# CSU-KangHu/HiTE

Hardware: AMD Instinct MI355X
Metric: candidate TE boundaries/sec on 1 Gbp synthetic genome (fine stage: copy finding+gather+align+vote+judge) (higher is better)
Workload: dtype u8; 1 GPU; C3: 1000 Mbp synthetic genome, 2500 TIR + 2500 LTR families, 50000 candidates/GPU judged as TIR (copy finding by minimizer-index lookup inside the timed step; index build 0.0 s untimed); genome_bp=1000000000, candidates_per_gpu=50000, candidate_bases=192511237, copies=799813, copy_table=found, is_te=34225, parallelism=replicated genome, candidates per rank x1, all-gather of 32-B calls

## Files before the change

hite_amd/csrc/hite_align.hip:

```cpp
#include "hite_common.h"
#include "hite_scan.h"
#include "hite_arena.h"
#include "hite_sort.h"
#include "hite_align.h"

#define AL_GAP 3
#define AL_STEER 24
#define AL_MARGIN 48
#define AL_PADR 1056
#define AL_WIDE_NW 64
#define AL_STRIP 16
#define AL_RECB 4096
#define AL_DEFAULT_CAP 8
#define AL_KBINS 2048
#define AL_LANES_MIN_STRIPS 32

struct AlignArgs {
    const uint8_t *win;
    const int64_t *win_off;
    const int32_t *win_len;
    const int32_t *row_first;
    int n_cand;
    const int32_t *row_cand;
    const uint4 *planes;
// ... 353 lines not shown
                    const int tr = m - H;
                    if (t + s > tr) s = (tr - t) & ~3;
                    const int need = tr - 3 - 8 * ((n - j) >> 2) - t;
                    if (s < need) s = (need + 3) & ~3;
                    if (s > 8) { status = 2; act = false; s = 8; }
                    if (!half) {
                        stop += plane_sum(X2[0], X1[0], X0[0], (1u << s) - 1u) - AL_GAP * s;
                        brec[(cc >> 2) * 2] = (uint32_t)(s >> 2) | (i2 << 2) | (i1 << 10) | (i0 << 18);
                    }
#pragma unroll
                    for (int w = 0; w < HW - 1; w++) {
                        X2[w] = alignbit(X2[w + 1], X2[w], (uint32_t)s); X1[w] = alignbit(X1[w + 1], X1[w], (uint32_t)s);
                        X0[w] = alignbit(X0[w + 1], X0[w], (uint32_t)s);
                        A0[w] = alignbit(A0[w + 1], A0[w], (uint32_t)s); A1[w] = alignbit(A1[w + 1], A1[w], (uint32_t)s);
                        AN[w] = alignbit(AN[w + 1], AN[w], (uint32_t)s);
                    }
                    X2[HW - 1] = alignbit(half ? 0xffffffffu : u2, X2[HW - 1], (uint32_t)s);
                    X1[HW - 1] = alignbit(half ? 0xffffffffu : u1, X1[HW - 1], (uint32_t)s);
                    X0[HW - 1] = alignbit(half ? 0u : u0, X0[HW - 1], (uint32_t)s);
                    A0[HW - 1] = alignbit(half ? f0 : ua0, A0[HW - 1], (uint32_t)s);
                    A1[HW - 1] = alignbit(half ? f1 : ua1, A1[HW - 1], (uint32_t)s);
                    AN[HW - 1] = alignbit(half ? fn : uan, AN[HW - 1], (uint32_t)s);
                    f0 >>= s; f1 >>= s; fn >>= s;
                    t += s;
                    if (t >= 1) { const int v = t + 1 - j; LO = v > LO ? v : LO; }
                    if (t + W < m) { const int jl = j + 3 < n ? j + 3 : n; const int v = t + W - jl; HI = v < HI ? v : HI; }
                }
            }
            const uint32_t word = cc < 4 ? bw.x : (cc < 8 ? bw.y : (cc < 12 ? bw.z : bw.w));
            const BaseMask bm = base_mask((word >> (8 * (cc & 3))) & 0xffu);
            uint32_t Bv[HW], Pv[HW], Yv[HW], Sv[HW], eqv[HW], vposv[HW];
#pragma unroll
            for (int w = 0; w < HW; w++) {
                eqv[w] = ~((A0[w] ^ bm.m0) | (A1[w] ^ bm.m1) | AN[w] | bm.inv);
                vposv[w] = X2[w] & X1[w];
                Bv[w] = eqv[w] | ~(X2[w] | X1[w] | X0[w]);
            }
            const uint32_t pvpos = pair_partner(vposv[HW - 1]);
            const uint32_t vin = half ? pvpos >> 31 : 0u;
            uint32_t cin = 0u, tap0 = 0u;
#pragma unroll
            for (int w = 0; w < HW; w++) {
                if (w == HW - 1) tap0 = cin;
                Pv[w] = (vposv[w] << 1) | (w ? vposv[w - 1] >> 31 : vin);
                Yv[w] = Pv[w] | Bv[w];
                unsigned cout;
                Sv[w] = __builtin_addc(Bv[w], Yv[w], cin, &cout);
                cin = cout;
            }
            {
                const uint32_t pc = pair_partner(cin);
                uint32_t e = half ? pc : 0u;
#pragma unroll
                for (int w = 0; w < HW; w++) { const uint32_t o = Sv[w]; Sv[w] = o + e; e &= (o == 0xffffffffu) ? 1u : 0u; }
            }
            uint32_t Zv[HW], h2v[HW], h1v[HW], h0v[HW];
#pragma unroll
            for (int w = 0; w < HW; w++) {
                Zv[w] = Bv[w] | (Pv[w] & (Sv[w] ^ Bv[w] ^ Yv[w]));
                const uint32_t b1 = Zv[w] & X0[w], b2 = X1[w] & b1;
                h0v[w] = ~(Zv[w] ^ X0[w]); h1v[w] = ~(X1[w] ^ b1); h2v[w] = ~(X2[w] ^ b2);
            }
            const uint32_t q2 = pair_partner(h2v[HW - 1]) >> 31, q1 = pair_partner(h1v[HW - 1]) >> 31, q0 = pair_partner(h0v[HW - 1]) >> 31;
            const uint32_t hin2 = half ? q2 : 1u, hin1 = half ? q1 : 1u, hin0 = half ? q0 : 0u;
            if (on) {
#pragma unroll
                for (int w = 0; w < HW; w++) {
                    const uint32_t s2 = (h2v[w] << 1) | (w ? h2v[w - 1] >> 31 : hin2), s1 = (h1v[w] << 1) | (w ? h1v[w - 1] >> 31 : hin1),
                                   s0 = (h0v[w] << 1) | (w ? h0v[w - 1] >> 31 : hin0);
                    const uint32_t c1 = Zv[w] & s0, c2 = s1 & c1;
                    X0[w] = ~(Zv[w] ^ s0); X1[w] = ~(s1 ^ c1); X2[w] = ~(s2 ^ c2);
                }
                if (!half) {
                    stop += AL_GAP;
                    const uint32_t c5 = tap0 | ((vposv[HW - 2] >> 31) << 1) | ((h2v[HW - 2] >> 31) << 2) | ((h1v[HW - 2] >> 31) << 3) | ((h0v[HW - 2] >> 31) << 4);
                    const int sh = 26 + 5 * (cc & 3);
                    if (sh + 5 <= 32) brec[(cc >> 2) * 2] |= c5 << sh;
                    else if (sh >= 32) brec[(cc >> 2) * 2 + 1] |= c5 << (sh - 32);
                    else { brec[(cc >> 2) * 2] |= c5 << sh; brec[(cc >> 2) * 2 + 1] |= c5 >> (32 - sh); }
                    brec[(cc >> 2) * 2 + 1] |= ((bm.m0 & 1u) | (bm.m1 & 2u) | (bm.inv & 4u)) << (14 + 3 * (cc & 3));
                }
            }
        }
        if (sa && !half) {
            uint4 *bp = reinterpret_cast<uint4 *>(rec0 + (size_t)k * AL_RECB + AL_RECB / 2);
            bp[0] = make_uint4(brec[0], brec[1], brec[2], brec[3]);
            bp[1] = make_uint4(brec[4], brec[5], brec[6], brec[7]);
        }
    }
    {
        const int extra = m - H - t;
        const uint32_t part = pair_partner((uint32_t)plane_sum(X2[0], X1[0], X0[0], (1u << (extra & 31)) - 1u));
        if (n > 0 && !half) {
            int U = -1, kstar = -1;
            if (status == 0) {
                int u = stop - AL_GAP * H;
#pragma unroll
                for (int w = 0; w < HW; w++) u += plane_sum(X2[w], X1[w], X0[w], 0xffffffffu);
                u += (int)part - AL_GAP * extra;
                U = u;
                const int d = m - n, dmin = d < 0 ? d : 0, dmax = d > 0 ? d : 0, ad = d < 0 ? -d : d;
                int E = dmin - LO;
                if (HI - dmax < E) E = HI - dmax;
                if (E > (1 << 27)) kstar = 0x7fffffff;
                else if (E >= 0) kstar = AL_GAP * ad + 2 * AL_GAP * E + 2 * AL_GAP - 1;
            }
            P.U[g] = U; P.kst[g] = kstar; P.st[g] = status; P.lvl[g] = NW;
        }
    }
}

template <int CTRL>
__device__ __forceinline__ uint32_t dpp_row(uint32_t v) { return (uint32_t)__builtin_amdgcn_update_dpp(0, (int)v, CTRL, 0xf, 0xf, true); }
template <int G>
__device__ __forceinline__ int grp_sum(int v) {
    v += (int)dpp_row<0xB1>((uint32_t)v);
    v += (int)dpp_row<0x4E>((uint32_t)v);
    if (G == 8) v += (int)dpp_row<0x141>((uint32_t)v);
    return v;
}
__device__ __forceinline__ int wave_min_i32(int v) {
#pragma unroll
    for (int d = 32; d >= 1; d >>= 1) { int o = __shfl_xor(v, d, 64); v = o < v ? o : v; }
    return v;
}
__device__ __forceinline__ uint32_t bit_mask(uint32_t w, int bit) { return (uint32_t)((int32_t)(w << (31 - bit)) >> 31); }
template <int GI>
__device__ __forceinline__ uint32_t quad_bcast(uint32_t v) { return dpp_row<GI * 0x55>(v); }
struct LaneFwd {
    uint32_t X2, X1, X0, A0, A1, AN, f0, f1, fn;
    int t, stop, LO, HI, status;
    bool act;
};
template <int G, bool FULL>
__device__ __forceinline__ void lanes_strip(LaneFwd &S, const uint4 bw, const uint32_t invm, const uint32_t code12, const bool sa, const int k,
                                            const int m, const int n, const int q, const uint32_t K1, const unsigned long long TOPM, uint32_t (&brec)[8]) {
    constexpr int NW = G, W = 32 * NW, H = W / 2, S0 = NW / 2 - 1;
    const bool top = q == G - 1;
#pragma unroll
    for (int cc = 0; cc < AL_STRIP; cc++) {
        const int j = k * AL_STRIP + cc + 1;
        const bool on = FULL || (sa && j <= n);
        if ((cc & 3) == 0) {
            const int ds = grp_sum<G>((q == S0 || q == S0 + 1) ? slope_count(S.X2, S.X1, S.X0) : 0);
            const uint32_t i2 = dpp_row<0x102>(S.X2) & 0xffu, i1 = dpp_row<0x102>(S.X1) & 0xffu, i0 = dpp_row<0x102>(S.X0) & 0xffu;
            const uint32_t u2 = dpp_row<0x101>(S.X2), u1 = dpp_row<0x101>(S.X1), u0 = dpp_row<0x101>(S.X0);
            const uint32_t ua0 = dpp_row<0x101>(S.A0), ua1 = dpp_row<0x101>(S.A1), uan = dpp_row<0x101>(S.AN);
            constexpr int gi = 0;
            const uint32_t cg = (cc >> 2) == 0 ? quad_bcast<0>(code12) : ((cc >> 2) == 1 ? quad_bcast<1>(code12) : ((cc >> 2) == 2 ? quad_bcast<2>(code12) : quad_bcast<3>(code12)));
            (void)gi;
            if (on) {
                int s = ds > AL_STEER ? 0 : (ds < -AL_STEER ? 8 : 4);
                const int tr = m - H;
                if (S.t + s > tr) s = (tr - S.t) & ~3;
                const int need = tr - 3 - 8 * ((n - j) >> 2) - S.t;
                if (s < need) s = (need + 3) & ~3;
                if (s > 8) { S.status = 2; S.act = false; s = 8; }
                S.stop += plane_sum(S.X2, S.X1, S.X0, (1u << s) - 1u) - AL_GAP * s;
                brec[(cc >> 2) * 2] = (uint32_t)(s >> 2) | (i2 << 2) | (i1 << 10) | (i0 << 18);
                brec[(cc >> 2) * 2 + 1] = cg << 14;
                S.X2 = alignbit(top ? 0xffffffffu : u2, S.X2, (uint32_t)s);
                S.X1 = alignbit(top ? 0xffffffffu : u1, S.X1, (uint32_t)s);
                S.X0 = alignbit(top ? 0u : u0, S.X0, (uint32_t)s);
                S.A0 = alignbit(top ? S.f0 : ua0, S.A0, (uint32_t)s);
                S.A1 = alignbit(top ? S.f1 : ua1, S.A1, (uint32_t)s);
                S.AN = alignbit(top ? S.fn : uan, S.AN, (uint32_t)s);
                S.f0 >>= s; S.f1 >>= s; S.fn >>= s;
                S.t += s;
                if (S.t >= 1) { const int v = S.t + 1 - j; S.LO = v > S.LO ? v : S.LO; }
                if (S.t + W < m) { const int jl = j + 3 < n ? j + 3 : n; const int v = S.t + W - jl; S.HI = v < S.HI ? v : S.HI; }
            }
        }
        const uint32_t word = cc < 4 ? bw.x : (cc < 8 ? bw.y : (cc < 12 ? bw.z : bw.w));
        const uint32_t m0 = bit_mask(word, 8 * (cc & 3) + 1), m1 = bit_mask(word, 8 * (cc & 3) + 2), inv = bit_mask(invm, cc);
        const uint32_t eq = ~((S.A0 ^ m0) | (S.A1 ^ m1) | S.AN | inv);
        const uint32_t vpos = S.X2 & S.X1;
        const uint32_t B = eq | ~(S.X2 | S.X1 | S.X0);
        const uint32_t pvr = dpp_row<0x111>(vpos);
        const uint32_t Pp = alignbit(vpos, pvr, 31) & ~K1;
        const uint32_t Y = Pp | B;
        unsigned long long Gm;
        const uint32_t sum0 = add_co_mask(B, Y, Gm);
        uint32_t sum;
        {
            const unsigned long long Pm = __ballot(sum0 == 0xffffffffu);
            const unsigned long long Gc = Gm & ~TOPM, Yy = (Pm | Gm) & ~TOPM, ss = Gc + Yy;
            sum = add_mask_bit(sum0, ss ^ Gc ^ Yy);
        }
        const uint32_t Z = B | (Pp & (sum ^ B ^ Y));
        const uint32_t h0 = ~(Z ^ S.X0), b1 = Z & S.X0, h1 = ~(S.X1 ^ b1), b2 = S.X1 & b1, h2 = ~(S.X2 ^ b2);
        const uint32_t r2 = dpp_row<0x111>(h2), r1 = dpp_row<0x111>(h1), r0 = dpp_row<0x111>(h0);
        if (on) {
            const uint32_t s2 = alignbit(h2, r2, 31) | K1, s1 = alignbit(h1, r1, 31) | K1, s0 = alignbit(h0, r0, 31) & ~K1;
            const uint32_t c1 = Z & s0, c2 = s1 & c1;
            S.X0 = ~(Z ^ s0); S.X1 = ~(s1 ^ c1); S.X2 = ~(s2 ^ c2);
            uint32_t c5 = alignbit(r0 >> 31, r1, 31);
            c5 = alignbit(c5, r2, 31);
            c5 = alignbit(c5, pvr, 31);
            c5 = (c5 << 1) | (sum - sum0);
            const int sh = 26 + 5 * (cc & 3);
            if (sh + 5 <= 32) brec[(cc >> 2) * 2] |= c5 << sh;
            else if (sh >= 32) brec[(cc >> 2) * 2 + 1] |= c5 << (sh - 32);
            else { brec[(cc >> 2) * 2] |= c5 << sh; brec[(cc >> 2) * 2 + 1] |= c5 >> (32 - sh); }
        }
    }
}
__device__ __forceinline__ uint32_t decode_bases4(uint32_t w) {
    uint32_t r = 0;
#pragma unroll
    for (int x = 0; x < 4; x++) {
        const unsigned ch = (w >> (8 * x)) & 0xffu;
        const uint32_t bad = is_acgt_byte(ch) ? 0u : 1u;
        r |= (bad << x) | ((((ch >> 1) & 3u) | (bad << 2)) << (4 + 3 * x));
    }
    return r;
}
template <int G>
__global__ void __launch_bounds__(64) align_fwd_lanes_kernel(AlignArgs P, const int32_t *__restrict__ list, int nlist) {
    constexpr int NW = G, W = 32 * NW, H = W / 2, S0 = NW / 2 - 1, PPW = 64 / G;
    const int q = threadIdx.x & (G - 1);
    const int li = blockIdx.x * PPW + (int)(threadIdx.x / G);
    const int g = li < nlist ? list[li] : -1;
    int m = 0, n = 0, g0 = 0, c = 0;
    if (g >= 0) {
        c = P.row_cand[g];
        g0 = P.row_first[c];
        if (g != g0) { m = P.win_len[g0]; n = P.win_len[g]; }
    }
    const int nmax = wave_max_i32(n);
    if (nmax == 0) return;
    const int nfull = wave_min_i32(n > 0 ? n : 0x7fffffff);
    const bool wr = q == S0;
    const uint32_t K1 = q == 0 ? 1u : 0u;
    const unsigned long long TOPM = G == 4 ? 0x8888888888888888ull : 0x8080808080808080ull;
    const uint8_t *b = P.win + (g >= 0 ? P.win_off[g] : 0);
    const uint4 *pl = P.planes + (g >= 0 ? P.plane_off[c] : 0);
    char *rec0 = g >= 0 ? reinterpret_cast<char *>(P.rec[g]) : nullptr;
    LaneFwd S;
    S.X2 = q >= NW / 2 ? 0xffffffffu : 0u; S.X1 = S.X2; S.X0 = 0u; S.A0 = 0u; S.A1 = 0u; S.AN = 0xffffffffu;
    S.f0 = S.f1 = S.fn = 0u;
    S.t = -H;
    S.act = n > 0;
    if (S.act) { const uint4 v = pl[((S.t + AL_PADR) >> 5) + q]; S.A0 = v.x; S.A1 = v.y; S.AN = v.z; }
    S.stop = AL_GAP * H; S.LO = -(1 << 28); S.HI = 1 << 28; S.status = 0;
    int fq = (S.t + W + AL_PADR) >> 5;
    uint4 Wa = make_uint4(0, 0, 0xffffffffu, 0), Wb = Wa, Wc = Wa, bnext = make_uint4(0, 0, 0, 0);
    if (S.act) { Wa = pl[fq]; Wb = pl[fq + 1]; Wc = pl[fq + 2]; bnext = *reinterpret_cast<const uint4 *>(b); }
    for (int k = 0; k * AL_STRIP < nmax; k++) {
        const bool sa = S.act && k * AL_STRIP < n;
        uint4 bw = make_uint4(0, 0, 0, 0);
        uint32_t brec[8] = {0, 0, 0, 0, 0, 0, 0, 0};
        {
            const uint32_t p2 = dpp_row<0x101>(S.X2), p1 = dpp_row<0x101>(S.X1), p0 = dpp_row<0x101>(S.X0);
            if (sa && wr) {
                uint4 *ck = reinterpret_cast<uint4 *>(rec0 + (size_t)k * AL_RECB);
                ck[0] = make_uint4(S.X2, p2, S.X1, p1);
                ck[1] = make_uint4(S.X0, p0, (uint32_t)(S.t + 32 * S0), 0u);
            }
        }
        S.f0 = S.f1 = S.fn = 0u;
        if (sa) {
            bw = bnext;
            if ((k + 1) * AL_STRIP < n) bnext = *reinterpret_cast<const uint4 *>(b + (k + 1) * AL_STRIP);
            const int fx = S.t + W + AL_PADR;
            if ((fx >> 5) != fq) { Wa = Wb; Wb = Wc; fq++; Wc = pl[fq + 2]; }
            const uint32_t sh = (uint32_t)fx & 31u;
            S.f0 = alignbit(Wb.x, Wa.x, sh); S.f1 = alignbit(Wb.y, Wa.y, sh); S.fn = alignbit(Wb.z, Wa.z, sh);
        }
        const uint32_t dq = (q & 3) == 0 ? bw.x : ((q & 3) == 1 ? bw.y : ((q & 3) == 2 ? bw.z : bw.w));
        const uint32_t dec = decode_bases4(dq);
        uint32_t invm = (dec & 15u) << (4 * (q & 3));
        invm |= dpp_row<0xB1>(invm);
        invm |= dpp_row<0x4E>(invm);
        const bool failed = __any(n > 0 && S.status != 0);
        if ((k + 1) * AL_STRIP <= nfull && !failed) lanes_strip<G, true>(S, bw, invm, dec >> 4, sa, k, m, n, q, K1, TOPM, brec);
        else lanes_strip<G, false>(S, bw, invm, dec >> 4, sa, k, m, n, q, K1, TOPM, brec);
        if (sa && wr) {
            uint4 *bp = reinterpret_cast<uint4 *>(rec0 + (size_t)k * AL_RECB + AL_RECB / 2);
            bp[0] = make_uint4(brec[0], brec[1], brec[2], brec[3]);
            bp[1] = make_uint4(brec[4], brec[5], brec[6], brec[7]);
        }
    }
    {
        const int extra = m - H - S.t;
        const int part = q < NW / 2 ? plane_sum(S.X2, S.X1, S.X0, 0xffffffffu) : (q == NW / 2 ? plane_sum(S.X2, S.X1, S.X0, (1u << (extra & 31)) - 1u) : 0);
        const int tot = grp_sum<G>(part + (q == 0 ? S.stop : 0));
        if (n > 0 && wr) {
            int U = -1, kstar = -1;
            if (S.status == 0) {
                U = tot + AL_GAP * n - AL_GAP * H - AL_GAP * extra;
                const int d = m - n, dmin = d < 0 ? d : 0, dmax = d > 0 ? d : 0, ad = d < 0 ? -d : d;
                int E = dmin - S.LO;
                if (S.HI - dmax < E) E = S.HI - dmax;
                if (E > (1 << 27)) kstar = 0x7fffffff;
                else if (E >= 0) kstar = AL_GAP * ad + 2 * AL_GAP * E + 2 * AL_GAP - 1;
            }
            P.U[g] = U; P.kst[g] = kstar; P.st[g] = S.status; P.lvl[g] = NW;
            if (NW == 4) P.U4[g] = U;
        }
    }
}

typedef unsigned int tb_u32x4 __attribute__((ext_vector_type(4)));
#if defined(ALIGN_TB_STORE8)
struct OpsOut {
    uint16_t *ops;
    unsigned long long acc, top;
    int m;
    __device__ __forceinline__ void init(uint16_t *row, int m_) { ops = row; m = m_; acc = 0ull; top = 0ull; }
    __device__ __forceinline__ void push(int pos, uint32_t val) {
        acc = (acc << 16) | (unsigned long long)(val & 0xffffu);
        if ((pos & 3) == 0) {
            if (pos + 4 <= m) *reinterpret_cast<unsigned long long *>(ops + pos) = acc;
            else top = acc;
        }
    }
    __device__ __forceinline__ void finish() {
        const int k = m & 3, p0 = m & ~3;
        for (int x = 0; x < k; x++) ops[p0 + x] = (uint16_t)(top >> (16 * x));
    }
};
#elif defined(ALIGN_TB_STORE32)
struct OpsOut {
    uint16_t *ops;
    unsigned long long acc;
    unsigned long long g0, g1, g2, g3;
    int m, off;
    int q_low;
    __device__ __forceinline__ void init(uint16_t *row, int m_) {
        ops = row; m = m_; acc = 0ull; g0 = g1 = g2 = g3 = 0ull;
        off = (int)((reinterpret_cast<uintptr_t>(row) >> 1) & 15);
        q_low = m_ + off;
    }
    __device__ __forceinline__ uint16_t held(int q, int q_acc_low) const {
        if ((q >> 2) == (q_acc_low >> 2) && (q_acc_low & 3)) return (uint16_t)(acc >> (16 * (q - q_acc_low)));
        const int g = (q >> 2) & 3;
        const unsigned long long s = g == 0 ? g0 : (g == 1 ? g1 : (g == 2 ? g2 : g3));
        return (uint16_t)(s >> (16 * (q & 3)));
    }
    __device__ __forceinline__ void push(int pos, uint32_t val) {
        acc = (acc << 16) | (unsigned long long)(val & 0xffffu);
        const int q = pos + off;
        if ((q & 3) == 0) {
            const int g = (q >> 2) & 3;
            g0 = g == 0 ? acc : g0; g1 = g == 1 ? acc : g1; g2 = g == 2 ? acc : g2; g3 = g == 3 ? acc : g3;
            if (g == 0) {
                if (pos + 16 <= m) {
                    tb_u32x4 *dst = reinterpret_cast<tb_u32x4 *>(ops + pos);
                    tb_u32x4 v0, v1;
                    v0.x = (unsigned)g0; v0.y = (unsigned)(g0 >> 32); v0.z = (unsigned)g1; v0.w = (unsigned)(g1 >> 32);
                    v1.x = (unsigned)g2; v1.y = (unsigned)(g2 >> 32); v1.z = (unsigned)g3; v1.w = (unsigned)(g3 >> 32);
                    dst[0] = v0; dst[1] = v1;
                } else {
                    for (int x = pos; x < m; x++) ops[x] = held(x + off, q);
                }
                q_low = q;
            }
        }
    }
    __device__ __forceinline__ void finish() {
        const int top = q_low - off < m ? q_low - off : m;
        for (int x = 0; x < top; x++) ops[x] = held(x + off, off);
    }
};

#else
struct OpsOut {
    uint16_t *ops;
    unsigned long long acc, hi;
    unsigned long long tacc, thi;
    int m, off;
    __device__ __forceinline__ void init(uint16_t *row, int m_) {
        ops = row; m = m_; acc = 0ull; hi = 0ull; tacc = 0ull; thi = 0ull;
        off = (int)((reinterpret_cast<uintptr_t>(row) >> 1) & 7);
    }
    __device__ __forceinline__ void push(int pos, uint32_t val) {
        acc = (acc << 16) | (unsigned long long)(val & 0xffffu);
        const int q = pos + off;
        if ((q & 3) == 0) {
            if (q & 4) hi = acc;
            else if (pos + 8 <= m) {
                tb_u32x4 v;
                v.x = (unsigned)acc; v.y = (unsigned)(acc >> 32); v.z = (unsigned)hi; v.w = (unsigned)(hi >> 32);
                *reinterpret_cast<tb_u32x4 *>(ops + pos) = v;
            } else { tacc = acc; thi = hi; }
        }
    }
    __device__ __forceinline__ void finish() {
        const int t0 = m - ((m + off) & 7);
        if (t0 >= 0) for (int x = t0; x < m; x++) { const int qq = x + off; ops[x] = (uint16_t)(((qq & 4) ? thi : tacc) >> (16 * (qq & 3))); }
        const int b0 = (8 - off) & 7;
        const int lowm = b0 < m ? b0 : m;
        for (int x = 0; x < lowm; x++) {
            const int qq = x + off;
            const bool in_acc = (off & 3) != 0 && (qq >> 2) == (off >> 2);
            ops[x] = in_acc ? (uint16_t)(acc >> (16 * x)) : (uint16_t)(hi >> (16 * (qq & 3)));
        }
    }
};
#endif

#ifdef ALIGN_TB_OCC
#define ALIGN_TB_ATTR __attribute__((amdgpu_waves_per_eu(ALIGN_TB_OCC, ALIGN_TB_OCC)))
#else
#define ALIGN_TB_ATTR
#endif
__global__ void __launch_bounds__(64) ALIGN_TB_ATTR align_tb_kernel(AlignArgs P, const int32_t *__restrict__ list, int nlist) {
    ACLK_BEGIN(1);
    const int li = blockIdx.x * 64 + threadIdx.x;
    const int g = li < nlist ? list[li] : -1;
    int m = 0, n = 0, g0 = 0, c = 0;
    if (g >= 0) {
        c = P.row_cand[g];
        g0 = P.row_first[c];
        if (g != g0 && P.st[g] == 0) { m = P.win_len[g0]; n = P.win_len[g]; }
    }
    const int nmax = wave_max_i32(n);
    if (nmax == 0) return;
    const uint4 *pl = P.planes + (g >= 0 ? P.plane_off[c] : 0);
    const char *rec0 = g >= 0 ? reinterpret_cast<const char *>(P.rec[g]) : nullptr;
    uint16_t *ops = P.ops + (g >= 0 ? P.ops_base[c] + (int64_t)(g - g0) * (m + 1) : 0);
    int i = m, j = n;
    bool fail = false;
    OpsOut out;
    out.init(ops, m);
    const int Kmax = (nmax + AL_STRIP - 1) / AL_STRIP;
    const int K = (n + AL_STRIP - 1) / AL_STRIP;
    struct Pw { uint32_t x, y, z; };
    uint4 ckA0, ckA1, ckB0, ckB1, bdA0, bdA1;
    Pw plA[4];
    ckA0 = ckA1 = ckB0 = ckB1 = bdA0 = bdA1 = make_uint4(0, 0, 0, 0);
#pragma unroll
    for (int w = 0; w < 4; w++) { plA[w].x = 0; plA[w].y = 0; plA[w].z = 0; }
    {
        const int k = Kmax - 1;
        if (k < K) {
            const uint4 *ck = reinterpret_cast<const uint4 *>(rec0 + (size_t)k * AL_RECB);
            ckA0 = ck[0]; ckA1 = ck[1];
            const uint4 *bp = reinterpret_cast<const uint4 *>(rec0 + (size_t)k * AL_RECB + AL_RECB / 2);
            bdA0 = bp[0]; bdA1 = bp[1];
            const int q0 = ((int)ckA1.z + AL_PADR) >> 5;
#pragma unroll
            for (int w = 0; w < 4; w++) { const uint4 v = pl[q0 + w]; plA[w].x = v.x; plA[w].y = v.y; plA[w].z = v.z; }
        }
        if (k >= 1 && k - 1 < K) {
            const uint4 *ck = reinterpret_cast<const uint4 *>(rec0 + (size_t)(k - 1) * AL_RECB);
            ckB0 = ck[0]; ckB1 = ck[1];
        }
    }
    for (int k = Kmax - 1; k >= 0; k--) {
        const bool sa = n > 0 && !fail && i > 0 && k < K;
        uint4 ckC0 = make_uint4(0, 0, 0, 0), ckC1 = ckC0, bdB0 = ckC0, bdB1 = ckC0;
        Pw plB[4];
#pragma unroll
        for (int w = 0; w < 4; w++) { plB[w].x = 0; plB[w].y = 0; plB[w].z = 0; }
        if (k >= 1 && k - 1 < K && !fail && i > 0) {
            const uint4 *bp = reinterpret_cast<const uint4 *>(rec0 + (size_t)(k - 1) * AL_RECB + AL_RECB / 2);
            bdB0 = bp[0]; bdB1 = bp[1];
            const int q0 = ((int)ckB1.z + AL_PADR) >> 5;
#pragma unroll
            for (int w = 0; w < 4; w++) { const uint4 v = pl[q0 + w]; plB[w].x = v.x; plB[w].y = v.y; plB[w].z = v.z; }
        }
        if (k >= 2 && k - 2 < K && !fail && i > 0) {
            const uint4 *ck = reinterpret_cast<const uint4 *>(rec0 + (size_t)(k - 2) * AL_RECB);
            ckC0 = ck[0]; ckC1 = ck[1];
        }
        if (__any(sa)) {
        uint32_t X2[2], X1[2], X0[2], A0[2], A1[2], AN[2];
        uint32_t f0 = 0, f1 = 0, fn = 0;
        uint32_t brec[8] = {0, 0, 0, 0, 0, 0, 0, 0};
        int t = 0;
        if (sa) {
            X2[0] = ckA0.x; X2[1] = ckA0.y; X1[0] = ckA0.z; X1[1] = ckA0.w; X0[0] = ckA1.x; X0[1] = ckA1.y;
            t = (int)ckA1.z;
            brec[0] = bdA0.x; brec[1] = bdA0.y; brec[2] = bdA0.z; brec[3] = bdA0.w;
            brec[4] = bdA1.x; brec[5] = bdA1.y; brec[6] = bdA1.z; brec[7] = bdA1.w;
            const uint32_t sh = (uint32_t)(t + AL_PADR) & 31u;
#pragma unroll
            for (int w = 0; w < 2; w++) {
                A0[w] = alignbit(plA[w + 1].x, plA[w].x, sh); A1[w] = alignbit(plA[w + 1].y, plA[w].y, sh);
                AN[w] = alignbit(plA[w + 1].z, plA[w].z, sh);
            }
            f0 = alignbit(plA[3].x, plA[2].x, sh); f1 = alignbit(plA[3].y, plA[2].y, sh); fn = alignbit(plA[3].z, plA[2].z, sh);
        } else {
#pragma unroll
            for (int w = 0; w < 2; w++) { X2[w] = 0; X1[w] = 0; X0[w] = 0; A0[w] = 0; A1[w] = 0; AN[w] = 0; }
        }
        unsigned long long dg[AL_STRIP], up[AL_STRIP];
        uint32_t sbits = 0;
#pragma unroll
        for (int cc = 0; cc < AL_STRIP; cc++) {
            const int jc = k * AL_STRIP + cc + 1;
            dg[cc] = 0ull; up[cc] = 0ull;
            if (sa && jc <= n) {
                const uint32_t rlo = brec[(cc >> 2) * 2], rhi = brec[(cc >> 2) * 2 + 1];
                if ((cc & 3) == 0) {
                    const uint32_t s = (rlo & 3u) << 2;
                    const uint32_t in2 = (rlo >> 2) & 0xffu, in1 = (rlo >> 10) & 0xffu, in0 = (rlo >> 18) & 0xffu;
                    X2[0] = alignbit(X2[1], X2[0], s); X1[0] = alignbit(X1[1], X1[0], s); X0[0] = alignbit(X0[1], X0[0], s);
                    A0[0] = alignbit(A0[1], A0[0], s); A1[0] = alignbit(A1[1], A1[0], s); AN[0] = alignbit(AN[1], AN[0], s);
                    X2[1] = alignbit(in2, X2[1], s); X1[1] = alignbit(in1, X1[1], s); X0[1] = alignbit(in0, X0[1], s);
                    A0[1] = alignbit(f0, A0[1], s); A1[1] = alignbit(f1, A1[1], s); AN[1] = alignbit(fn, AN[1], s);
                    f0 >>= s; f1 >>= s; fn >>= s;
                    t += (int)s;
                    sbits |= (rlo & 3u) << (2 * (cc >> 2));
                }
                const int sh = 26 + 5 * (cc & 3);
                const uint32_t c5 = (sh + 5 <= 32 ? rlo >> sh : (sh >= 32 ? rhi >> (sh - 32) : (rlo >> sh) | (rhi << (32 - sh)))) & 31u;
                const uint32_t code = rhi >> (14 + 3 * (cc & 3));
                BaseMask bm;
                bm.m0 = 0u - (code & 1u); bm.m1 = 0u - ((code >> 1) & 1u); bm.inv = 0u - ((code >> 2) & 1u);
                uint32_t tap[5], dgc[2], upc[2];
                bp_core<2, true, -1>(X2, X1, X0, A0, A1, AN, bm, c5 & 1u, (c5 >> 1) & 1u, (c5 >> 2) & 1u, (c5 >> 3) & 1u, (c5 >> 4) & 1u, dgc, upc, tap);
                dg[cc] = ((unsigned long long)dgc[1] << 32) | dgc[0];
                up[cc] = ((unsigned long long)upc[1] << 32) | upc[0];
            }
        }
        int tcur = t;
#pragma unroll
        for (int cc = AL_STRIP - 1; cc >= 0; cc--) {
            const int jc = k * AL_STRIP + cc + 1;
            if (sa && !fail && i > 0 && j == jc) {
                const int kb = i - tcur - 1;
                if ((unsigned)kb >= 64u) fail = true;
                else {
                    const unsigned long long stopm = (dg[cc] | ~up[cc]) & (0xffffffffffffffffull >> (63 - kb));
                    if (stopm == 0ull) fail = true;
                    else {
                        const int ps = 63 - __clzll(stopm);
                        int ups = kb - ps;
                        if (ups > i) ups = i;
                        const uint32_t gapv = (uint32_t)j | 0x8000u;
                        for (int x = 0; x < ups; x++) out.push(i - 1 - x, gapv);
                        i -= ups;
                        if (i > 0) {
                            if ((dg[cc] >> ps) & 1ull) { out.push(i - 1, (uint32_t)(j - 1)); i--; j--; }
                            else j--;
                        }
                    }
                }
            }
            if ((cc & 3) == 0) tcur -= (int)(((sbits >> (2 * (cc >> 2))) & 3u) << 2);
        }
        }
        ckA0 = ckB0; ckA1 = ckB1; ckB0 = ckC0; ckB1 = ckC1; bdA0 = bdB0; bdA1 = bdB1;
#pragma unroll
        for (int w = 0; w < 4; w++) plA[w] = plB[w];
    }
    if (n > 0) {
        if (fail) P.st[g] = 1;
        else {
            for (int q = i - 1; q >= 0; q--) out.push(q, 0x8000u);
            out.finish();
        }
    }
    ACLK_END();
}

__device__ __forceinline__ uint32_t lane_above(uint32_t v, uint32_t fill) { return (uint32_t)__builtin_amdgcn_update_dpp((int)fill, (int)v, 0x130, 0xf, 0xf, false); }
__device__ __forceinline__ uint32_t lane_below(uint32_t v, uint32_t fill) { return (uint32_t)__builtin_amdgcn_update_dpp((int)fill, (int)v, 0x138, 0xf, 0xf, false); }
__device__ __forceinline__ int wave_sum_i32(int v) {
#pragma unroll
    for (int d = 32; d >= 1; d >>= 1) v += __shfl_xor(v, d, 64);
    return v;
}

__device__ __forceinline__ uint32_t lane_below_keep(uint32_t v, uint32_t &keep) {
    asm volatile("s_nop 1\n\tv_mov_b32_dpp %0, %1 wave_shr:1 row_mask:0xf bank_mask:0xf" : "+v"(keep) : "v"(v));
    return keep;
}
__device__ __forceinline__ void lane_below_keep3(uint32_t v2, uint32_t v1, uint32_t v0, uint32_t &k2, uint32_t &k1, uint32_t &k0) {
    asm volatile("s_nop 1\n\tv_mov_b32_dpp %0, %3 wave_shr:1 row_mask:0xf bank_mask:0xf\n\tv_mov_b32_dpp %1, %4 wave_shr:1 row_mask:0xf bank_mask:0xf\n\t"
                 "v_mov_b32_dpp %2, %5 wave_shr:1 row_mask:0xf bank_mask:0xf" : "+v"(k2), "+v"(k1), "+v"(k0) : "v"(v2), "v"(v1), "v"(v0));
}
struct WideFwd {
    uint32_t X2, X1, X0, A0, A1, AN, f0, f1, fn;
    uint32_t kz0, kz1, ko0, ko1;
    int t, stop, LO, HI, status;
};
template <bool FULL>
__device__ __forceinline__ void wide_fwd_strip(WideFwd &S, const AlignArgs &P, int lane, int m, int n, int j0, int64_t full0, unsigned long long M0,
                                               unsigned long long M1, unsigned long long MI) {
    constexpr int NW = AL_WIDE_NW, W = 32 * NW, H = W / 2, S0 = NW / 2 - 1;
    uint32_t *fb = P.fullbuf + (full0 + j0) * (2 * NW) + lane;
#pragma unroll
    for (int cc = 0; cc < AL_STRIP; cc++) {
        const int j = j0 + cc;
        if (FULL || (j <= n && S.status == 0)) {
            if ((cc & 3) == 0) {
                const int dv = slope_count(S.X2, S.X1, S.X0);
                const int ds = __builtin_amdgcn_readlane(dv, S0) + __builtin_amdgcn_readlane(dv, S0 + 1);
                int s = ds > AL_STEER ? 0 : (ds < -AL_STEER ? 8 : 4);
                const int tr = m - H;
                if (S.t + s > tr) s = (tr - S.t) & ~3;
                const int need = tr - 3 - 8 * ((n - j) >> 2) - S.t;
                if (s < need) s = (need + 3) & ~3;
                if (s > 8) { S.status = 2; s = 8; }
                const uint32_t smask = (1u << s) - 1u;
                S.stop += plane_sum((uint32_t)__builtin_amdgcn_readlane((int)S.X2, 0), (uint32_t)__builtin_amdgcn_readlane((int)S.X1, 0),
                                    (uint32_t)__builtin_amdgcn_readlane((int)S.X0, 0), smask) - AL_GAP * s;
                S.X2 = alignbit(lane_above(S.X2, 0xffffffffu), S.X2, (uint32_t)s);
                S.X1 = alignbit(lane_above(S.X1, 0xffffffffu), S.X1, (uint32_t)s);
                S.X0 = alignbit(lane_above(S.X0, 0u), S.X0, (uint32_t)s);
                S.A0 = alignbit(lane_above(S.A0, S.f0), S.A0, (uint32_t)s);
                S.A1 = alignbit(lane_above(S.A1, S.f1), S.A1, (uint32_t)s);
                S.AN = alignbit(lane_above(S.AN, S.fn), S.AN, (uint32_t)s);
                S.f0 >>= s; S.f1 >>= s; S.fn >>= s;
                S.t += s;
                if (S.t >= 1) { const int v = S.t + 1 - j; S.LO = v > S.LO ? v : S.LO; }
                if (S.t + W < m) { const int jl = j + 3 < n ? j + 3 : n; const int v = S.t + W - jl; S.HI = v < S.HI ? v : S.HI; }
                if (lane < 4 && j + lane <= n) P.fullt[full0 + j + lane] = S.t;
            }
            S.stop += AL_GAP;
            BaseMask bm;
            bm.m0 = 0u - (uint32_t)((M0 >> cc) & 1ull); bm.m1 = 0u - (uint32_t)((M1 >> cc) & 1ull); bm.inv = 0u - (uint32_t)((MI >> cc) & 1ull);
            const uint32_t eq = ~((S.A0 ^ bm.m0) | (S.A1 ^ bm.m1) | S.AN | bm.inv);
            const uint32_t vneg = ~(S.X2 | S.X1 | S.X0), vpos = S.X2 & S.X1;
            const uint32_t B = eq | vneg, Pp = alignbit(vpos, lane_below_keep(vpos, S.kz0), 31);
            const uint32_t Y = Pp | B;
            unsigned long long Gm;
            uint32_t sum = add_co_mask(B, Y, Gm);
            {
                const unsigned long long Pm = __ballot(sum == 0xffffffffu);
                const unsigned long long Yy = Pm | Gm, ss = Gm + Yy;
                const unsigned long long into = ss ^ Gm ^ Yy;
                sum = add_mask_bit(sum, into);
            }
            const uint32_t Z = B | (Pp & (sum ^ B ^ Y));
            const uint32_t h0 = ~(Z ^ S.X0), b1 = Z & S.X0, h1 = ~(S.X1 ^ b1), b2 = S.X1 & b1, h2 = ~(S.X2 ^ b2);
            lane_below_keep3(h2, h1, h0, S.ko0, S.ko1, S.kz1);
            const uint32_t s2 = alignbit(h2, S.ko0, 31), s1 = alignbit(h1, S.ko1, 31), s0 = alignbit(h0, S.kz1, 31);
            const uint32_t n0 = ~(Z ^ s0), c1 = Z & s0, n1 = ~(s1 ^ c1), c2 = s1 & c1, n2 = ~(s2 ^ c2);
            S.X2 = n2; S.X1 = n1; S.X0 = n0;
            fb[cc * (2 * NW)] = eq | ~Z;
            fb[cc * (2 * NW) + NW] = n2 & n1;
        }
    }
}
__global__ void __launch_bounds__(64) align_wide_fwd_kernel(AlignArgs P, const int32_t *__restrict__ list, int nlist) {
    constexpr int NW = AL_WIDE_NW, W = 32 * NW, H = W / 2;
    const int pi = blockIdx.x;
    if (pi >= nlist) return;
    const int lane = threadIdx.x;
    const int g = list[pi];
    const int c = P.row_cand[g], g0 = P.row_first[c];
    if (g == g0) return;
    const int m = P.win_len[g0], n = P.win_len[g];
    const uint8_t *b = P.win + P.win_off[g];
    const uint4 *pl = P.planes + P.plane_off[c];
    const int64_t full0 = P.full_off[g];
    WideFwd S;
    S.t = -H;
    S.X2 = lane >= NW / 2 ? 0xffffffffu : 0u; S.X1 = S.X2; S.X0 = 0u;
    { const uint4 v = pl[((S.t + AL_PADR) >> 5) + lane]; S.A0 = v.x; S.A1 = v.y; S.AN = v.z; }
    S.stop = AL_GAP * H; S.LO = -(1 << 28); S.HI = 1 << 28; S.status = 0;
    S.kz0 = 0u; S.kz1 = 0u; S.ko0 = 0x80000000u; S.ko1 = 0x80000000u;
    unsigned chn = b[lane & 15];
    for (int j0 = 1; j0 <= n && S.status == 0; j0 += AL_STRIP) {
        const unsigned ch = chn;
        chn = b[j0 - 1 + AL_STRIP + (lane & 15)];
        const unsigned long long M0 = __ballot((ch >> 1) & 1u), M1 = __ballot((ch >> 2) & 1u), MI = __ballot(!is_acgt_byte(ch));
        {
            const int fx = S.t + W + AL_PADR;
            const uint4 F = pl[fx >> 5], G = pl[(fx >> 5) + 1];
            const uint32_t sh = (uint32_t)fx & 31u;
            S.f0 = alignbit(G.x, F.x, sh); S.f1 = alignbit(G.y, F.y, sh); S.fn = alignbit(G.z, F.z, sh);
        }
        if (j0 + AL_STRIP - 1 <= n) wide_fwd_strip<true>(S, P, lane, m, n, j0, full0, M0, M1, MI);
        else wide_fwd_strip<false>(S, P, lane, m, n, j0, full0, M0, M1, MI);
    }
    int U = -1, kstar = -1;
    if (S.status == 0) {
        const int extra = m - H - S.t;
        U = S.stop - AL_GAP * H - AL_GAP * extra +
            wave_sum_i32(lane < NW / 2 ? plane_sum(S.X2, S.X1, S.X0, 0xffffffffu) : (lane == NW / 2 ? plane_sum(S.X2, S.X1, S.X0, (1u << extra) - 1u) : 0));
        const int d = m - n, dmin = d < 0 ? d : 0, dmax = d > 0 ? d : 0, ad = d < 0 ? -d : d;
        int E = dmin - S.LO;
        if (S.HI - dmax < E) E = S.HI - dmax;
        if (E > (1 << 27)) kstar = 0x7fffffff;
        else if (E >= 0) kstar = AL_GAP * ad + 2 * AL_GAP * E + 2 * AL_GAP - 1;
    }
    if (lane == 0) { P.U[g] = U; P.kst[g] = kstar; P.st[g] = S.status; P.lvl[g] = NW | 0x100; }
}

struct WideOps {
    uint16_t *ops;
    int m, lane;
    uint32_t acc;
    __device__ __forceinline__ void flush(int base) { if (base + lane < m) ops[base + lane] = (uint16_t)acc; }
    __device__ __forceinline__ void put(int pos, uint32_t val) {
        if (lane == (pos & 63)) acc = val;
        if ((pos & 63) == 0) flush(pos);
    }
    __device__ __forceinline__ void run_diag(int hi, int count, int delta) {
        while (count > 0) {
            const int base = hi & ~63;
            const int lo = hi - count + 1 > base ? hi - count + 1 : base;
            if (base + lane >= lo && base + lane <= hi) acc = (uint32_t)(base + lane + delta);
            const int k = hi - lo + 1;
            count -= k; hi -= k;
            if (lo == base) flush(base);
        }
    }
    __device__ __forceinline__ void run(int hi, int count, uint32_t val) {
        while (count > 0) {
            const int base = hi & ~63;
            const int lo = hi - count + 1 > base ? hi - count + 1 : base;
            if (base + lane >= lo && base + lane <= hi) acc = val;
            const int k = hi - lo + 1;
            count -= k; hi -= k;
            if (lo == base) flush(base);
        }
    }
};
__global__ void __launch_bounds__(64) align_wide_tb_kernel(AlignArgs P, const int32_t *__restrict__ list, int nlist) {
    constexpr int NW = AL_WIDE_NW, W = 32 * NW, PF = 8;
    const int pi = blockIdx.x;
    if (pi >= nlist) return;
    const int lane = threadIdx.x;
    const int g = list[pi];
    const int c = P.row_cand[g], g0 = P.row_first[c];
    if (g == g0 || P.st[g] != 0) return;
    const int m = P.win_len[g0], n = P.win_len[g];
    WideOps out;
    out.ops = P.ops + P.ops_base[c] + (int64_t)(g - g0) * (m + 1); out.m = m; out.lane = lane; out.acc = 0u;
    const int64_t full0 = P.full_off[g];
    int i = m, j = n;
    bool fail = false;
    uint32_t dgn[PF];
    int ttn[PF];
#pragma unroll
    for (int q = 0; q < PF; q++) {
        const int jq = j - q > 0 ? j - q : 1;
        dgn[q] = P.fullbuf[(full0 + jq) * (2 * NW) + lane]; ttn[q] = P.fullt[full0 + jq];
    }
    while (i > 0 && j > 0 && !fail) {
        uint32_t dgs[PF];
        int tts[PF];
#pragma unroll
        for (int q = 0; q < PF; q++) { dgs[q] = dgn[q]; tts[q] = ttn[q]; }
#pragma unroll
        for (int q = 0; q < PF; q++) {
            const int jq = j - PF - q > 0 ? j - PF - q : 1;
            dgn[q] = P.fullbuf[(full0 + jq) * (2 * NW) + lane]; ttn[q] = P.fullt[full0 + jq];
        }
#pragma unroll
        for (int q = 0; q < PF; q++) {
            if (i > 0 && j > 0 && !fail) {
                const uint32_t dgw = dgs[q];
                const int kb = i - tts[q] - 1;
                if ((unsigned)kb >= (unsigned)W) fail = true;
                else {
                    const int wq = kb >> 5;
                    const uint32_t dcur = (uint32_t)__builtin_amdgcn_readlane((int)dgw, wq);
                    if ((dcur >> (kb & 31)) & 1u) { out.put(i - 1, (uint32_t)(j - 1)); i--; j--; }
                    else {
                        const uint32_t upw = P.fullbuf[(full0 + j) * (2 * NW) + NW + lane];
                        const uint32_t low = 0xffffffffu >> (31 - (kb & 31));
                        const uint32_t sbit = dgw | ~upw;
                        const uint32_t mk = lane > wq ? 0u : (lane == wq ? sbit & low : sbit);
                        const unsigned long long nz = __ballot(mk != 0u);
                        if (nz == 0ull) fail = true;
                        else {
                            const int tl = 63 - __clzll(nz);
                            const uint32_t mt = (uint32_t)__builtin_amdgcn_readlane((int)mk, tl), dt = (uint32_t)__builtin_amdgcn_readlane((int)dgw, tl);
                            const int ps = 32 * tl + 31 - __clz(mt);
                            int nup = kb - ps;
                            if (nup > i) nup = i;
                            out.run(i - 1, nup, (uint32_t)j | 0x8000u);
                            i -= nup;
                            if (i > 0) {
                                if ((dt >> (ps & 31)) & 1u) { out.put(i - 1, (uint32_t)(j - 1)); i--; j--; }
                                else j--;
                            }
                        }
                    }
                }
            }
        }
    }
    if (fail) { if (lane == 0) P.st[g] = 1; }
    else out.run(i - 1, i, 0x8000u);
}

__device__ __forceinline__ unsigned long long readlane_u64(unsigned long long v, int l) {
    return ((unsigned long long)(uint32_t)__builtin_amdgcn_readlane((int)(uint32_t)(v >> 32), l) << 32) | (uint32_t)__builtin_amdgcn_readlane((int)(uint32_t)v, l);
}
__global__ void __launch_bounds__(64) align_tb_strips_kernel(AlignArgs P, const int32_t *__restrict__ list, int nlist) {
    __shared__ unsigned long long s_dg[64][AL_STRIP + 1], s_up[64][AL_STRIP + 1];
    __shared__ int s_t[64][4];
    const int pi = blockIdx.x;
    if (pi >= nlist) return;
    const int lane = threadIdx.x;
    const int g = list[pi];
    const int c = P.row_cand[g], g0 = P.row_first[c];
    if (g == g0 || P.st[g] != 0) return;
    const int m = P.win_len[g0], n = P.win_len[g];
    if (n <= 0) return;
    const uint4 *pl = P.planes + P.plane_off[c];
    const char *rec0 = reinterpret_cast<const char *>(P.rec[g]);
    WideOps out;
    out.ops = P.ops + P.ops_base[c] + (int64_t)(g - g0) * (m + 1); out.m = m; out.lane = lane; out.acc = 0u;
    const int K = (n + AL_STRIP - 1) / AL_STRIP;
    int i = m, j = n;
    bool fail = false;
    for (int kb0 = K - 1; kb0 >= 0 && !fail && i > 0; kb0 -= 64) {
        {
            const int k = kb0 - lane;
            if (k >= 0) {
                const uint4 *ck = reinterpret_cast<const uint4 *>(rec0 + (size_t)k * AL_RECB);
                const uint4 *bp = reinterpret_cast<const uint4 *>(rec0 + (size_t)k * AL_RECB + AL_RECB / 2);
                const uint4 ck0 = ck[0], ck1 = ck[1], bd0 = bp[0], bd1 = bp[1];
                uint32_t X2[2] = {ck0.x, ck0.y}, X1[2] = {ck0.z, ck0.w}, X0[2] = {ck1.x, ck1.y}, A0[2], A1[2], AN[2];
                int t = (int)ck1.z;
                const uint32_t brec[8] = {bd0.x, bd0.y, bd0.z, bd0.w, bd1.x, bd1.y, bd1.z, bd1.w};
                const int q0 = (t + AL_PADR) >> 5;
                const uint4 p0 = pl[q0], p1 = pl[q0 + 1], p2 = pl[q0 + 2], p3 = pl[q0 + 3];
                const uint32_t sh = (uint32_t)(t + AL_PADR) & 31u;
                A0[0] = alignbit(p1.x, p0.x, sh); A1[0] = alignbit(p1.y, p0.y, sh); AN[0] = alignbit(p1.z, p0.z, sh);
                A0[1] = alignbit(p2.x, p1.x, sh); A1[1] = alignbit(p2.y, p1.y, sh); AN[1] = alignbit(p2.z, p1.z, sh);
                uint32_t f0 = alignbit(p3.x, p2.x, sh), f1 = alignbit(p3.y, p2.y, sh), fn = alignbit(p3.z, p2.z, sh);
#pragma unroll
                for (int cc = 0; cc < AL_STRIP; cc++) {
                    const int jc = k * AL_STRIP + cc + 1;
                    unsigned long long dgv = 0ull, upv = 0ull;
                    if (jc <= n) {
                        const uint32_t rlo = brec[(cc >> 2) * 2], rhi = brec[(cc >> 2) * 2 + 1];
                        if ((cc & 3) == 0) {
                            const uint32_t s = (rlo & 3u) << 2;
                            const uint32_t in2 = (rlo >> 2) & 0xffu, in1 = (rlo >> 10) & 0xffu, in0 = (rlo >> 18) & 0xffu;
                            X2[0] = alignbit(X2[1], X2[0], s); X1[0] = alignbit(X1[1], X1[0], s); X0[0] = alignbit(X0[1], X0[0], s);
                            A0[0] = alignbit(A0[1], A0[0], s); A1[0] = alignbit(A1[1], A1[0], s); AN[0] = alignbit(AN[1], AN[0], s);
                            X2[1] = alignbit(in2, X2[1], s); X1[1] = alignbit(in1, X1[1], s); X0[1] = alignbit(in0, X0[1], s);
                            A0[1] = alignbit(f0, A0[1], s); A1[1] = alignbit(f1, A1[1], s); AN[1] = alignbit(fn, AN[1], s);
                            f0 >>= s; f1 >>= s; fn >>= s;
                            t += (int)s;
                        }
                        const int sh5 = 26 + 5 * (cc & 3);
                        const uint32_t c5 = (sh5 + 5 <= 32 ? rlo >> sh5 : (sh5 >= 32 ? rhi >> (sh5 - 32) : (rlo >> sh5) | (rhi << (32 - sh5)))) & 31u;
                        const uint32_t code = rhi >> (14 + 3 * (cc & 3));
                        BaseMask bm;
                        bm.m0 = 0u - (code & 1u); bm.m1 = 0u - ((code >> 1) & 1u); bm.inv = 0u - ((code >> 2) & 1u);
                        uint32_t tap[5], dgc[2], upc[2];
                        bp_core<2, true, -1>(X2, X1, X0, A0, A1, AN, bm, c5 & 1u, (c5 >> 1) & 1u, (c5 >> 2) & 1u, (c5 >> 3) & 1u, (c5 >> 4) & 1u, dgc, upc, tap);
                        dgv = ((unsigned long long)dgc[1] << 32) | dgc[0];
                        upv = ((unsigned long long)upc[1] << 32) | upc[0];
                    }
                    s_dg[lane][cc] = dgv; s_up[lane][cc] = upv;
                    if ((cc & 3) == 0) s_t[lane][cc >> 2] = t;
                }
            }
        }
        __syncthreads();
        const int nst = kb0 + 1 < 64 ? kb0 + 1 : 64;
        unsigned long long dgn = s_dg[0][lane & 15], upn = s_up[0][lane & 15];
        int tn = s_t[0][(lane & 15) >> 2];
        for (int l = 0; l < nst && !fail && i > 0; l++) {
            const unsigned long long dgl = dgn, upl = upn;
// ... 499 lines not shown
```

Measured before the change: 655,700 candidates/s.

## Make alignment traceback branch-free with batched gap-run writes across the wave

Rewrites the traceback output buffer as four 32-bit words and adds a run() method that shifts in up to eight identical gap ops at once, so long vertical gap runs and the final leading gaps are emitted in 8-op chunks instead of one push per op. The per-column traceback step becomes predicated and wave-uniform (loop bound nmax made scalar via readfirstlane), which removes divergent branches and serial per-lane loops. It also drops the alternative STORE8/STORE32 output variants and adds an optional run-count debug counter. The cost is extra predicated ALU work on inactive lanes and more complex shift/select logic.

```diff
diff --git a/hite_amd/csrc/hite_align.hip b/hite_amd/csrc/hite_align.hip
--- a/hite_amd/csrc/hite_align.hip
+++ b/hite_amd/csrc/hite_align.hip
@@ -679,102 +679,80 @@
 }
 
 typedef unsigned int tb_u32x4 __attribute__((ext_vector_type(4)));
-#if defined(ALIGN_TB_STORE8)
 struct OpsOut {
     uint16_t *ops;
-    unsigned long long acc, top;
-    int m;
-    __device__ __forceinline__ void init(uint16_t *row, int m_) { ops = row; m = m_; acc = 0ull; top = 0ull; }
-    __device__ __forceinline__ void push(int pos, uint32_t val) {
-        acc = (acc << 16) | (unsigned long long)(val & 0xffffu);
-        if ((pos & 3) == 0) {
-            if (pos + 4 <= m) *reinterpret_cast<unsigned long long *>(ops + pos) = acc;
-            else top = acc;
-        }
-    }
-    __device__ __forceinline__ void finish() {
-        const int k = m & 3, p0 = m & ~3;
-        for (int x = 0; x < k; x++) ops[p0 + x] = (uint16_t)(top >> (16 * x));
-    }
-};
-#elif defined(ALIGN_TB_STORE32)
-struct OpsOut {
-    uint16_t *ops;
-    unsigned long long acc;
-    unsigned long long g0, g1, g2, g3;
-    int m, off;
-    int q_low;
-    __device__ __forceinline__ void init(uint16_t *row, int m_) {
-        ops = row; m = m_; acc = 0ull; g0 = g1 = g2 = g3 = 0ull;
-        off = (int)((reinterpret_cast<uintptr_t>(row) >> 1) & 15);
-        q_low = m_ + off;
-    }
-    __device__ __forceinline__ uint16_t held(int q, int q_acc_low) const {
-        if ((q >> 2) == (q_acc_low >> 2) && (q_acc_low & 3)) return (uint16_t)(acc >> (16 * (q - q_acc_low)));
-        const int g = (q >> 2) & 3;
-        const unsigned long long s = g == 0 ? g0 : (g == 1 ? g1 : (g == 2 ? g2 : g3));
-        return (uint16_t)(s >> (16 * (q & 3)));
-    }
-    __device__ __forceinline__ void push(int pos, uint32_t val) {
-        acc = (acc << 16) | (unsigned long long)(val & 0xffffu);
-        const int q = pos + off;
-        if ((q & 3) == 0) {
-            const int g = (q >> 2) & 3;
-            g0 = g == 0 ? acc : g0; g1 = g == 1 ? acc : g1; g2 = g == 2 ? acc : g2; g3 = g == 3 ? acc : g3;
-            if (g == 0) {
-                if (pos + 16 <= m) {
-                    tb_u32x4 *dst = reinterpret_cast<tb_u32x4 *>(ops + pos);
-                    tb_u32x4 v0, v1;
-                    v0.x = (unsigned)g0; v0.y = (unsigned)(g0 >> 32); v0.z = (unsigned)g1; v0.w = (unsigned)(g1 >> 32);
-                    v1.x = (unsigned)g2; v1.y = (unsigned)(g2 >> 32); v1.z = (unsigned)g3; v1.w = (unsigned)(g3 >> 32);
-                    dst[0] = v0; dst[1] = v1;
-                } else {
-                    for (int x = pos; x < m; x++) ops[x] = held(x + off, q);
-                }
-                q_low = q;
-            }
-        }
-    }
-    __device__ __forceinline__ void finish() {
-        const int top = q_low - off < m ? q_low - off : m;
-        for (int x = 0; x < top; x++) ops[x] = held(x + off, off);
-    }
-};
-
-#else
-struct OpsOut {
-    uint16_t *ops;
-    unsigned long long acc, hi;
-    unsigned long long tacc, thi;
+    uint32_t w[4];
+    uint32_t tw[4];
     int m, off;
     __device__ __forceinline__ void init(uint16_t *row, int m_) {
-        ops = row; m = m_; acc = 0ull; hi = 0ull; tacc = 0ull; thi = 0ull;
+        ops = row; m = m_;
+#pragma unroll
+        for (int k = 0; k < 4; k++) { w[k] = 0u; tw[k] = 0u; }
         off = (int)((reinterpret_cast<uintptr_t>(row) >> 1) & 7);
     }
-    __device__ __forceinline__ void push(int pos, uint32_t val) {
-        acc = (acc << 16) | (unsigned long long)(val & 0xffffu);
-        const int q = pos + off;
-        if ((q & 3) == 0) {
-            if (q & 4) hi = acc;
-            else if (pos + 8 <= m) {
-                tb_u32x4 v;
-                v.x = (unsigned)acc; v.y = (unsigned)(acc >> 32); v.z = (unsigned)hi; v.w = (unsigned)(hi >> 32);
-                *reinterpret_cast<tb_u32x4 *>(ops + pos) = v;
-            } else { tacc = acc; thi = hi; }
-        }
+    __device__ __forceinline__ void chunk(bool edge, int pe) {
+        if (edge && pe + 8 <= m) {
+            tb_u32x4 v;
+            v.x = w[0]; v.y = w[1]; v.z = w[2]; v.w = w[3];
+            *reinterpret_cast<tb_u32x4 *>(ops + pe) = v;
+        }
+        if (edge && pe + 8 > m) {
+#pragma unroll
+            for (int k = 0; k < 4; k++) tw[k] = w[k];
+        }
+    }
+    __device__ __forceinline__ void shift_in(int c, uint32_t r2) {
+        const int u = (c + 1) >> 1;
+        const uint32_t sv = (uint32_t)(c & 1) << 4;
+        uint32_t T[5];
+#pragma unroll
+        for (int k = 0; k < 5; k++) {
+            uint32_t x = r2;
+#pragma unroll
+            for (int uu = 0; uu <= k; uu++) x = u == uu ? w[k - uu < 4 ? k - uu : 3] : x;
+            T[k] = x;
+        }
+#pragma unroll
+        for (int k = 0; k < 4; k++) w[k] = alignbit(T[k + 1], T[k], sv);
+    }
+    __device__ __forceinline__ void run(int top, int cnt, uint32_t val) {
+        const int qlo = top - cnt + 1 + off;
+        const int a = (-qlo) & 7;
+        const bool cross = a < cnt;
+        const int c1 = cross ? cnt - a : cnt;
+        const uint32_t r2 = val | (val << 16);
+        shift_in(c1, r2);
+        chunk(cross, qlo + a - off);
+        shift_in(cnt - c1, r2);
+    }
+    __device__ __forceinline__ void push(bool en, int pos, uint32_t val) {
+        const uint32_t n3 = alignbit(w[3], w[2], 16u), n2 = alignbit(w[2], w[1], 16u), n1 = alignbit(w[1], w[0], 16u), n0 = (w[0] << 16) | val;
+        w[3] = en ? n3 : w[3]; w[2] = en ? n2 : w[2]; w[1] = en ? n1 : w[1]; w[0] = en ? n0 : w[0];
+        chunk(en && ((pos + off) & 7) == 0, pos);
     }
     __device__ __forceinline__ void finish() {
         const int t0 = m - ((m + off) & 7);
-        if (t0 >= 0) for (int x = t0; x < m; x++) { const int qq = x + off; ops[x] = (uint16_t)(((qq & 4) ? thi : tacc) >> (16 * (qq & 3))); }
+        if (t0 >= 0) for (int x = t0; x < m; x++) ops[x] = slot(tw, x - t0);
         const int b0 = (8 - off) & 7;
         const int lowm = b0 < m ? b0 : m;
-        for (int x = 0; x < lowm; x++) {
-            const int qq = x + off;
-            const bool in_acc = (off & 3) != 0 && (qq >> 2) == (off >> 2);
-            ops[x] = in_acc ? (uint16_t)(acc >> (16 * x)) : (uint16_t)(hi >> (16 * (qq & 3)));
-        }
+        for (int x = 0; x < lowm; x++) ops[x] = slot(w, x);
+    }
+    static __device__ __forceinline__ uint16_t slot(const uint32_t (&v)[4], int s) {
+        const uint32_t x = s < 2 ? v[0] : (s < 4 ? v[1] : (s < 6 ? v[2] : v[3]));
+        return (uint16_t)(x >> (16 * (s & 1)));
     }
 };
+
+#ifdef ALIGN_TB_RUNCOUNT
+__device__ unsigned long long g_tb_runs[2];
+extern "C" int hite_debug_align_tb_runs(unsigned long long *out) {
+    if (hipMemcpyFromSymbol(out, HIP_SYMBOL(g_tb_runs), 2 * sizeof(unsigned long long), 0) != hipSuccess) return -1;
+    const unsigned long long z[2] = {0ull, 0ull};
+    return hipMemcpyToSymbol(HIP_SYMBOL(g_tb_runs), z, sizeof z, 0) == hipSuccess ? 0 : -1;
+}
+#define TB_RUNCOUNT(k, v) do { if (threadIdx.x == 0) atomicAdd(&g_tb_runs[k], (unsigned long long)(v)); } while (0)
+#else
+#define TB_RUNCOUNT(k, v) do { } while (0)
 #endif
 
 #ifdef ALIGN_TB_OCC
@@ -792,7 +770,7 @@
         g0 = P.row_first[c];
         if (g != g0 && P.st[g] == 0) { m = P.win_len[g0]; n = P.win_len[g]; }
     }
-    const int nmax = wave_max_i32(n);
+    const int nmax = __builtin_amdgcn_readfirstlane(wave_max_i32(n));
     if (nmax == 0) return;
     const uint4 *pl = P.planes + (g >= 0 ? P.plane_off[c] : 0);
     const char *rec0 = g >= 0 ? reinterpret_cast<const char *>(P.rec[g]) : nullptr;
@@ -844,32 +822,23 @@
         }
         if (__any(sa)) {
         uint32_t X2[2], X1[2], X0[2], A0[2], A1[2], AN[2];
-        uint32_t f0 = 0, f1 = 0, fn = 0;
-        uint32_t brec[8] = {0, 0, 0, 0, 0, 0, 0, 0};
-        int t = 0;
-        if (sa) {
-            X2[0] = ckA0.x; X2[1] = ckA0.y; X1[0] = ckA0.z; X1[1] = ckA0.w; X0[0] = ckA1.x; X0[1] = ckA1.y;
-            t = (int)ckA1.z;
-            brec[0] = bdA0.x; brec[1] = bdA0.y; brec[2] = bdA0.z; brec[3] = bdA0.w;
-            brec[4] = bdA1.x; brec[5] = bdA1.y; brec[6] = bdA1.z; brec[7] = bdA1.w;
-            const uint32_t sh = (uint32_t)(t + AL_PADR) & 31u;
-#pragma unroll
-            for (int w = 0; w < 2; w++) {
-                A0[w] = alignbit(plA[w + 1].x, plA[w].x, sh); A1[w] = alignbit(plA[w + 1].y, plA[w].y, sh);
-                AN[w] = alignbit(plA[w + 1].z, plA[w].z, sh);
-            }
-            f0 = alignbit(plA[3].x, plA[2].x, sh); f1 = alignbit(plA[3].y, plA[2].y, sh); fn = alignbit(plA[3].z, plA[2].z, sh);
-        } else {
-#pragma unroll
-            for (int w = 0; w < 2; w++) { X2[w] = 0; X1[w] = 0; X0[w] = 0; A0[w] = 0; A1[w] = 0; AN[w] = 0; }
-        }
+        X2[0] = ckA0.x; X2[1] = ckA0.y; X1[0] = ckA0.z; X1[1] = ckA0.w; X0[0] = ckA1.x; X0[1] = ckA1.y;
+        int t = (int)ckA1.z;
+        const uint32_t brec[8] = {bdA0.x, bdA0.y, bdA0.z, bdA0.w, bdA1.x, bdA1.y, bdA1.z, bdA1.w};
+        const uint32_t sh0 = (uint32_t)(t + AL_PADR) & 31u;
+#pragma unroll
+        for (int w = 0; w < 2; w++) {
+            A0[w] = alignbit(plA[w + 1].x, plA[w].x, sh0); A1[w] = alignbit(plA[w + 1].y, plA[w].y, sh0);
+            AN[w] = alignbit(plA[w + 1].z, plA[w].z, sh0);
+        }
+        uint32_t f0 = alignbit(plA[3].x, plA[2].x, sh0), f1 = alignbit(plA[3].y, plA[2].y, sh0), fn = alignbit(plA[3].z, plA[2].z, sh0);
         unsigned long long dg[AL_STRIP], up[AL_STRIP];
         uint32_t sbits = 0;
 #pragma unroll
         for (int cc = 0; cc < AL_STRIP; cc++) {
             const int jc = k * AL_STRIP + cc + 1;
             dg[cc] = 0ull; up[cc] = 0ull;
-            if (sa && jc <= n) {
+            if (jc <= nmax) {
                 const uint32_t rlo = brec[(cc >> 2) * 2], rhi = brec[(cc >> 2) * 2 + 1];
                 if ((cc & 3) == 0) {
                     const uint32_t s = (rlo & 3u) << 2;
@@ -897,25 +866,35 @@
 #pragma unroll
         for (int cc = AL_STRIP - 1; cc >= 0; cc--) {
             const int jc = k * AL_STRIP + cc + 1;
-            if (sa && !fail && i > 0 && j == jc) {
+            if (jc <= nmax) {
+                const bool act = sa && !fail && i > 0 && j == jc;
                 const int kb = i - tcur - 1;
-                if ((unsigned)kb >= 64u) fail = true;
-                else {
-                    const unsigned long long stopm = (dg[cc] | ~up[cc]) & (0xffffffffffffffffull >> (63 - kb));
-                    if (stopm == 0ull) fail = true;
-                    else {
-                        const int ps = 63 - __clzll(stopm);
-                        int ups = kb - ps;
-                        if (ups > i) ups = i;
-                        const uint32_t gapv = (uint32_t)j | 0x8000u;
-                        for (int x = 0; x < ups; x++) out.push(i - 1 - x, gapv);
-                        i -= ups;
-                        if (i > 0) {
-                            if ((dg[cc] >> ps) & 1ull) { out.push(i - 1, (uint32_t)(j - 1)); i--; j--; }
-                            else j--;
-                        }
+                const unsigned long long stopm = (dg[cc] | ~up[cc]) & (0xffffffffffffffffull >> ((63 - kb) & 63));
+                const bool ok = act && (unsigned)kb < 64u && stopm != 0ull;
+                fail = fail || (act && !ok);
+                const int ps = 63 - __clzll(stopm | 1ull);
+                int ups = kb - ps;
+                ups = ups > i ? i : ups;
+                const int i2 = i - ups;
+                const bool dstep = ok && i2 > 0 && ((dg[cc] >> ps) & 1ull);
+                const uint32_t gapv = (uint32_t)j | 0x8000u;
+                int r = ok ? ups : 0, top = i - 1;
+                TB_RUNCOUNT(0, 1);
+                if (__any(r > 0)) {
+                    if (__any(r > 7)) {
+                        TB_RUNCOUNT(1, 1);
+                        do {
+                            const bool e8 = r > 7;
+                            out.run(top, e8 ? 8 : 0, gapv);
+                            r -= e8 ? 8 : 0; top -= e8 ? 8 : 0;
+                        } while (__any(r > 7));
                     }
+                    out.run(top, r, gapv);
+                    top -= r;
                 }
+                out.push(dstep, top, (uint32_t)(j - 1));
+                i = ok ? i2 - (dstep ? 1 : 0) : i;
+                j = ok && i2 > 0 ? j - 1 : j;
             }
             if ((cc & 3) == 0) tcur -= (int)(((sbits >> (2 * (cc >> 2))) & 3u) << 2);
         }
@@ -926,11 +905,14 @@
     }
     if (n > 0) {
         if (fail) P.st[g] = 1;
-        else {
-            for (int q = i - 1; q >= 0; q--) out.push(q, 0x8000u);
-            out.finish();
-        }
-    }
+    }
+    int r = n > 0 && !fail ? i : 0;
+    while (__any(r > 0)) {
+        const int cnt = r < 8 ? r : 8;
+        out.run(r - 1, cnt, 0x8000u);
+        r -= cnt;
+    }
+    if (n > 0 && !fail) out.finish();
     ACLK_END();
 }
 
```

Result: no change. 658,700 candidates/s (median of 5 runs) (+0.5%).
